# thiery-lab/manifold-mcmc-for-diffusions

Hardware: AMD Instinct MI355X
Metric: constrained-leapfrog steps/sec (all chains), FHN noisy-obs 400 sub-steps (higher is better)
Workload: dtype f64; 1 GPU; FHN noisy-obs, T=100 obs, S=400 steps/obs, R=5 obs/subseq, sigma_y=0.1, 256 chains per GPU (BASELINE.json configs[1]), Newton solver, standard splitting; chains_per_gpu=256, global_chains=256, dim_q=80106, traj_len=16, stepping=chmc_leapfrog_steps per trajectory (batched steps), chain_steps_nominal=152320, parallelism=chains x1 (no data-path collective, 1 gather), ranks_joined=1, collective_world_size=1, collective_route=torch.distributed gather, overlap_halves=-1

## Files before the change

### manifold_mcmc_for_diffusions_amd/csrc/backend_hip.h

```cpp
#pragma once
#include <hip/hip_runtime.h>

static thread_local hipStream_t g_stream = nullptr;
static thread_local hipStream_t g_streams[3] = {nullptr, nullptr, nullptr};
static thread_local int g_device = -1;
static hipError_t g_first_err = hipSuccess;

static inline void note(hipError_t e) {
  if (e != hipSuccess && g_first_err == hipSuccess) g_first_err = e;
}
static int dev_set(int device) {
  hipError_t e = hipSetDevice(device);
  if (e != hipSuccess) {
    g_err = std::string("hipSetDevice: ") + hipGetErrorString(e);
    return -1;
  }
  return 0;
}
static int dev_init(int device) {
  int n = 0;
  hipError_t e = hipGetDeviceCount(&n);
  if (e != hipSuccess || n <= 0) {
    g_err = std::string("no HIP device available (") + hipGetErrorString(e) + ")";
    return -1;
// ... 248 lines not shown
    partial[((size_t)c * gridDim.x + blockIdx.x) * nacc + threadIdx.x] =
        (sm[0][threadIdx.x] + sm[1][threadIdx.x]) + (sm[2][threadIdx.x] + sm[3][threadIdx.x]);
}
static int rowsum_groups(int ncol) { return ((ncol + 1) / 2 + 256 * CHMC_ROWSUM_PAIRS - 1) / (256 * CHMC_ROWSUM_PAIRS); }
template <class F>
static void launch_rowsum(F f, int ncol, int B, int nacc, double* partial, int cls = 0) {
  if (ncol <= 0 || B <= 0) return;
  (void)cls;
  hipLaunchKernelGGL(k_rowsum<F>, dim3((unsigned)rowsum_groups(ncol), (unsigned)B), dim3(256), 0, g_stream, f, ncol, nacc,
                     partial);
  note(hipGetLastError());
}
template <class F>
__global__ void __launch_bounds__(256) k_colmax(F f, int ncol, int rev) {
  const int c = rev ? gridDim.y - 1 - blockIdx.y : blockIdx.y;
  if (!f.active(c)) return;
  const int col = blockIdx.x * 256 + threadIdx.x;
  unsigned long long v = 0ULL;
  if (col < ncol) v = f(c, col);
  unsigned long long* tgt = f.red(c);
  if (!tgt) return;
  for (int off = 32; off > 0; off >>= 1) {
    const unsigned long long o = __shfl_xor(v, off, 64);
    v = o > v ? o : v;
  }
  __shared__ unsigned long long sm[4];
  if ((threadIdx.x & 63) == 0) sm[threadIdx.x >> 6] = v;
  __syncthreads();
  if (threadIdx.x == 0) {
    for (int i = 1; i < 4; ++i) v = sm[i] > v ? sm[i] : v;
    if (v) atomicMax(tgt, v);
  }
}
static thread_local unsigned* g_publish_ticket = nullptr;
template <class F>
static void launch_publish(F f, long n, int* counter, int poll_slot) {
  if (n <= 0) return;
  if (!g_poll_host) {
    note(hipHostMalloc((void**)&g_poll_host, 4 * sizeof(int), hipHostMallocDefault));
    for (int i = 0; i < 4; ++i) note(hipEventCreateWithFlags(&g_poll_ev[i], hipEventDisableTiming));
  }
  if (!g_publish_ticket) {
    note(hipMalloc((void**)&g_publish_ticket, 4 * sizeof(unsigned)));
    note(hipMemset(g_publish_ticket, 0, 4 * sizeof(unsigned)));
  }
  ProfRec r;
  const bool prof = g_prof_on_for(0);
  if (prof) {
    r.a = prof_event(), r.b = prof_event(), r.cls = 0;
    note(hipEventRecord(r.a, g_stream));
  }
  hipLaunchKernelGGL(k_run_publish<F>, dim3((unsigned)((n + 255) / 256)), dim3(256), 0, g_stream, f, (int)n, counter,
                     g_poll_host + poll_slot, g_publish_ticket + poll_slot);
  note(hipGetLastError());
  if (prof) {
    note(hipEventRecord(r.b, g_stream));
    g_prof_pending.push_back(r);
    if (g_prof_pending.size() > 4096) prof_drain();
  }
  note(hipEventRecord(g_poll_ev[poll_slot], g_stream));
}
template <class F>
static void launch_colmax(F f, int ncol, int B, int cls = 0) {
  if (ncol <= 0 || B <= 0) return;
  ProfRec r;
  const bool prof = g_prof_on_for(cls);
  if (prof) {
    r.a = prof_event(), r.b = prof_event(), r.cls = cls;
    note(hipEventRecord(r.a, g_stream));
  }
  hipLaunchKernelGGL(k_colmax<F>, dim3((unsigned)((ncol + 255) / 256), (unsigned)B), dim3(256), 0, g_stream, f, ncol,
                     next_chain_direction());
  note(hipGetLastError());
  if (prof) {
    note(hipEventRecord(r.b, g_stream));
    g_prof_pending.push_back(r);
    if (g_prof_pending.size() > 4096) prof_drain();
  }
}
template <class K, class... Args>
static void launch_wave(K kern, long nwaves, int cls, Args... args) {
  if (nwaves <= 0) return;
  ProfRec r;
  const bool prof = g_prof_on_for(cls);
  if (prof) {
    r.a = prof_event(), r.b = prof_event(), r.cls = cls;
    note(hipEventRecord(r.a, g_stream));
  }
  const int wpb = 1;
  note_forward_launch();
  hipLaunchKernelGGL(kern, dim3((unsigned)((nwaves + wpb - 1) / wpb)), dim3(64 * wpb), 0, g_stream, args...);
  note(hipGetLastError());
  if (prof) {
    note(hipEventRecord(r.b, g_stream));
    g_prof_pending.push_back(r);
    if (g_prof_pending.size() > 4096) prof_drain();
  }
}
template <class K, class... Args>
static void launch_blocks(K kern, long nblocks, int bs, int cls, Args... args) {
  if (nblocks <= 0) return;
  ProfRec r;
  const bool prof = g_prof_on_for(cls);
  if (prof) {
    r.a = prof_event(), r.b = prof_event(), r.cls = cls;
    note(hipEventRecord(r.a, g_stream));
  }
  hipLaunchKernelGGL(kern, dim3((unsigned)nblocks), dim3(bs), 0, g_stream, args...);
  note(hipGetLastError());
  if (prof) {
    note(hipEventRecord(r.b, g_stream));
    g_prof_pending.push_back(r);
// ... 23 lines not shown
```

### manifold_mcmc_for_diffusions_amd/csrc/chmc_api.inc

```
#include <string>
#include <algorithm>
#include <vector>
#include <cstring>
#include <cstdio>
#include <cstdlib>
#include <cmath>
#include <thread>
#include <type_traits>
#include "../../include/chmc.h"
#include "chmc_plan.h"
#include "chmc_layout.h"

using namespace chmc;

static thread_local std::string g_err;
static int fail(const std::string& m) {
  g_err = m;
  return -1;
}
#include CHMC_BACKEND_HEADER

struct chmc_ctx : ChainView {
  std::thread::id owner = std::this_thread::get_id();
  chmc_config cfg;
// ... 372 lines not shown
    launch(KSymBlk<M, RM>{sy, c->sl, c->w, which, 0}, (long)sy.B * sy.K, 9);
    solve_chain<M, RM, 1, 1>(sy, c->sl, c->w, which, 0, psel);
    jt_lambda<M, RM, 1>(c, which, 0, psel);
  });
}

static void iteration_scan(chmc_ctx* c, int newton, int prev, int qsel, int fwd_guess, int use_nw) {
  dispatch(c, [&](auto inst) {
    c->diag[7] += fwd<typename decltype(inst)::M, decltype(inst)::RM>(c, prev ^ 1, qsel, use_nw, newton ? 2 : 0, fwd_guess);
  });
}
static void iteration_scan_pair(chmc_ctx* c, int newton, int prev, int qsel, const Work& w1) {
  dispatch(c, [&](auto inst) {
    c->diag[7] += fwd_pair<typename decltype(inst)::M, decltype(inst)::RM>(c, w1, prev ^ 1, qsel, newton ? 2 : 0);
  });
  c->diag[6]++;
}
static void iteration_after_scan(chmc_ctx* c, int newton, int prev, int qsel) {
  const Sys& sy = c->sy;
  dispatch(c, [&](auto inst) {
    using M = typename decltype(inst)::M;
    constexpr int RM = decltype(inst)::RM;
    bool solved = false;
    if (newton) {
      solved = newton_sweep<M, RM>(c, prev, qsel);
      if (!solved) solve_chain<M, RM, 0, 0>(sy, c->sl, c->w, prev, qsel, 0);
    } else {
      launch(KSymBlk<M, RM>{sy, c->sl, c->w, prev, 1}, (long)sy.B * sy.K, 9);
      solve_chain<M, RM, 1, 0>(sy, c->sl, c->w, prev, qsel, 0);
    }
    jt_lambda<M, RM, 0>(c, prev, qsel, 0, solved);
  });
}

static int retract_waves(const chmc_ctx* c, int newton, const void* views) {
  return chain_kernel_waves(c->plan, part_plan(c).retract_chain && chain_kernel_model(c), c->sy.B, c->num_cus, newton != 0,
                            views != nullptr);
}
static int traj_waves(const chmc_ctx* c, int n_inner, int newton) {
  const bool eligible = part_plan(c).traj_chain && chain_kernel_model(c) && n_inner == 1 && c->mom_tangent && c->halves == 1;
  return chain_kernel_waves(c->plan, eligible, c->sy.B, c->num_cus, newton != 0, false);
}
static int run_projection(chmc_ctx* c, int newton, int prev, int qsel, double ctol, double ptol, double dtol,
                          int max_iters, const ViewSave* views = nullptr, int count_dir = -1) {
  const Sys& sy = c->sy;
  auto iters_dst = [&] { return count_dir < 0 ? nullptr : (count_dir ? c->d_itb : c->d_itf); };
  if (const int waves = retract_waves(c, newton, views)) {
    dispatch(c, [&](auto inst) {
      retract_chain<typename decltype(inst)::M, decltype(inst)::RM>(waves, (long)sy.B, sy, c->sl, c->w, prev, qsel, ctol, ptol,
                                                                     dtol, max_iters, iters_dst());
    });
    c->counters[6]++;
    c->diag[2]++;
    return 0;
  }
  const int nh = views ? 2 : 1;
  auto enter = [&](int h) {
    if (views) set_half(c, *views, h);
  };
  for (int h = 0; h < nh; ++h) {
    enter(h);
    if (sy.B > 0) launch(KNewtonBegin{c->w}, sy.B);
  }
  int fwd_guess = 2;
  const bool carry = c->plan.fwd == FwdPar && sy.K == 1;
  const int max_rounds = carry ? 12 * (max_iters + 1) : max_iters;
// ... 72 lines not shown
  w.Dw = alloc<double>(c, B * KM * RM * RM), w.JuL = alloc<double>(c, B * KM * RM * U), w.zbP = alloc<double>(c, B * KM * RM * Z);
  if (c->plan.pb_allocated) {
    w.muF = alloc<double>(c, B * ivls * X);
    w.ivl = alloc<double>(c, B * ivls * (2 * X * X + X * Z));
  }
  w.err = alloc<double>(c, B), w.ndq = alloc<unsigned long long>(c, B);
  w.iters = alloc<int>(c, B), w.nw = alloc<int>(c, B), w.nstat = alloc<int>(c, B), w.ok = alloc<int>(c, B), w.status = alloc<int>(c, B);
  w.n_active = alloc<int>(c, 4);
  c->d_itf_next = alloc<int>(c, B);
  c->have_pair = true;
}

static int run_projection_pair(chmc_ctx* c, int newton, double ctol, double ptol, double dtol, int max_iters) {
  const Sys& sy = c->sy;
  const int prev = 1, qsel = 1;
  const Work wk[2] = {c->w, c->pw};
  int* const iters_dst[2] = {c->d_itb, c->d_itf_next};
  const int dir[2] = {1, 0};
  auto enter = [&](int p) { c->w = wk[p]; };
  bool done[2], predict[2], stopped[2] = {false, false};
  int rounds_done[2] = {0, 0};
  for (int p = 0; p < 2; ++p) {
    enter(p);
    launch(KNewtonBegin{c->w}, sy.B);
    done[p] = sy.B <= 0;
    predict[p] = c->proj_stable[dir[p]] >= 3 && c->proj_rounds[dir[p]] >= 2;
  }
  for (int it = 0; it < max_iters && !(done[0] && done[1]); ++it) {
    for (int p = 0; p < 2; ++p)
      if (!done[p] && predict[p] && it >= c->proj_rounds[dir[p]] && poll_end(2 * p + ((it - 1) & 1)) == 0)
        done[p] = stopped[p] = true;
    if (done[0] && done[1]) break;
    c->round = it;
    if (!done[0] && !done[1]) {
      enter(0);
      iteration_scan_pair(c, newton, prev, qsel, wk[1]);
    } else {
      enter(done[0] ? 1 : 0);
      iteration_scan(c, newton, prev, qsel, it == 0 ? 2 : 1, 1);
    }
    for (int p = 0; p < 2; ++p) {
      if (done[p]) continue;
      enter(p);
      iteration_after_scan(c, newton, prev, qsel);
      const KCheck chk{c->w, ctol, ptol, dtol, max_iters, sy.B, iters_dst[p], it & 3};
      if (it >= 1) launch_publish(chk, sy.B, c->w.n_active + (it & 3), 2 * p + (it & 1));
      else launch(chk, sy.B);
      c->counters[6]++, c->diag[8]++;
    }
    if (it == 0) continue;
    for (int p = 0; p < 2; ++p) {
      if (done[p]) continue;
      if (it >= 2 && poll_end(2 * p + ((it - 1) & 1)) == 0) {
        done[p] = true;
        c->counters[6]--;
        continue;
      }
      rounds_done[p] = it + 1;
      if (it + 1 >= max_iters) poll_end(2 * p + (it & 1));
    }
  }
  for (int p = 0; p < 2; ++p) {
    int& expect = c->proj_rounds[dir[p]];
    int& stable = c->proj_stable[dir[p]];
    if (stopped[p] && rounds_done[p] < expect) rounds_done[p] = expect;
    stable = rounds_done[p] == expect ? stable + 1 : 0;
    expect = rounds_done[p];
    enter(p);
    if (sy.B > 0) launch(KNewtonEnd{c->w, iters_dst[p]}, sy.B);
  }
  enter(0);
  c->round = 0;
  return 0;
}

static int check_ctx(const chmc_ctx* c, const char* fn) {
  if (!c) return fail(std::string(fn) + ": null context");
// ... 1312 lines not shown
```

### manifold_mcmc_for_diffusions_amd/csrc/chmc_core.h

```cpp
#pragma once
#include <math.h>
#include <stdint.h>
#include "chmc_model.h"

#define CHMC_FI __attribute__((always_inline))
#if defined(__HIPCC__)
#define CHMC_UNROLL _Pragma("unroll")
#define CHMC_UNROLL4 _Pragma("unroll 4")
#else
#define CHMC_UNROLL
#define CHMC_UNROLL4
#endif

namespace chmc {

#ifndef CHMC_FWD_DEPTH
#define CHMC_FWD_DEPTH 4
#endif
#define CHMC_Q_PAD 256
#define CHMC_TPAD 16

struct BlockDesc {
  int obs0, nobs, first, last;
  int row0, nrows, ny;
// ... 1616 lines not shown
        const double* lam = w.lampad + ((size_t)c * sy.Kmax + b) * RM;
        const double* lam2 = w.lampad2 + ((size_t)c * sy.Kmax + b) * RM;
        const double* Jv = pick(sl.Jv, s) + (size_t)c * RM * sy.NV + col;
        const int nr = sy.blk[b].nrows;
        for (int i = 0; i < RM; ++i)
          if (i < nr) {
            const double jv = Jv[(size_t)i * sy.NV];
            d += jv * lam[i];
            if (TGT == 3) d2 += jv * lam2[i];
          }
      } else {
        const int t = e - sy.V0;
        col = sy.NV + t;
        const int b = sy.obs2blk[t];
        const int j = t - sy.blk[b].obs0;
        if (j < sy.blk[b].ny) {
          const double sg = sigma_at(sy, pick(sl.q, s) + (size_t)c * sy.Q);
          d = sg * w.lampad[((size_t)c * sy.Kmax + b) * RM + j];
          if (TGT == 3) d2 = sg * w.lampad2[((size_t)c * sy.Kmax + b) * RM + j];
        }
      }
      if (TGT == 0) r = absbits(d);
      const double gn = tgt[col] - d;
      tgt[col] = gn;
      if (TGT == 3) {
        const double pn = tgt2[col] - d2;
        tgt2[col] = pn;
        if (flow_rev) rev_flow1(c, s, off + col, pn, gn);
      }
    }
    return r;
  }
};

template <class M>
struct KInitInterp {
  Sys sy;
  double* q;
  const double* u;
  const double* v0;
  const double* xobs;
  CHMC_HD void operator()(int tid) const {
    constexpr int X = M::X, V = M::V;
    static_assert(X == V, "the interpolation solve needs a square noise matrix");
    const int TS = sy.T * sy.S;
    const int c = tid / TS, s = tid - c * TS;
    const int t = s / sy.S, i = s - t * sy.S;
    double* qc = q + (size_t)c * sy.Q;
    const double* uc = u + (size_t)c * sy.U;
    ChainConsts<M> cc;
    cc.init(uc, sy.dl);
    double xa[X], xs[X], dlt[X], f0[X], zero[V], A[X * X], Bm[X * V], rhs[X];
    if (t == 0) {
      M::gx0(cc.z, v0 + (size_t)c * sy.V0, xa);
    } else {
      for (int a = 0; a < X; ++a) xa[a] = xobs[((size_t)c * sy.T + t - 1) * X + a];
    }
    for (int a = 0; a < X; ++a) {
      dlt[a] = (xobs[((size_t)c * sy.T + t) * X + a] - xa[a]) / sy.S;
      xs[a] = xa[a] + i * dlt[a];
    }
    for (int a = 0; a < V; ++a) zero[a] = 0.0;
    M::step(cc.k, xs, zero, f0);
    M::jac_ab(cc.k, xs, zero, A, Bm);
    for (int a = 0; a < X; ++a) rhs[a] = dlt[a] - (f0[a] - xs[a]);
    int piv[X];
// ... 1076 lines not shown
```

### manifold_mcmc_for_diffusions_amd/csrc/chmc_passes.inc

```

static_assert(SirModel::ID == CHMC_MODEL_SIR && SirVsModel::ID == CHMC_MODEL_SIR && FhnModel::ID == CHMC_MODEL_FHN &&
                  FhnVsModel::ID == CHMC_MODEL_FHN && FhnNbModel::ID == CHMC_MODEL_FHN_NOTEBOOK,
              "chain_kernel_model and kChainKernels gate the per-chain kernels on the same models");
static bool chain_kernel_model(const chmc_ctx* c) { return c->model == CHMC_MODEL_SIR; }
template <class M, int RM>
constexpr bool kChainKernels = RM == 16 && M::ID == CHMC_MODEL_SIR;

template <int RM, int TGT>
static void update(const Sys& sy, const Slots& sl, const Work& w, int which, int qsel, int psel) {
  if (sy.Q % 2 == 0 && sy.NV % 2 == 0 && sy.U % 2 == 0 && sy.V0 % 2 == 0 && sy.V % 2 == 0 && sy.NCOL % 2 == 0)
    launch_colmax(KUpdate<RM, TGT, 2>{sy, sl, w, which, qsel, psel}, sy.NCOL / 2, sy.B, 4);
  else
    launch_colmax(KUpdate<RM, TGT, 1>{sy, sl, w, which, qsel, psel}, sy.NCOL, sy.B, 4);
}
template <class M, int RM, int TGT>
static void jt_lambda(chmc_ctx* c, int which, int qsel, int psel, bool have_mu_f = false, int flow_rev = 0,
                      double* fwd_qb = nullptr, double fwd_hfrac = 0.0) {
  const Sys& sy = c->sy;
  if (c->plan.rows != RowsCompact) return update<RM, TGT>(sy, c->sl, c->w, which, qsel, psel);
  if (!have_mu_f) launch(KMuF<RM, M::X, TGT>{sy, c->sl, c->w, which}, (long)sy.B * sy.K * sy.NOBS * M::X, 5);
  launch_colmax(KUpdatePB<RM, M::X, M::V, TGT>{sy, c->sl, c->w, which, qsel, psel, flow_rev, fwd_qb, fwd_hfrac},
                sy.T * sy.S + sy.V0 + (sy.noisy ? sy.T : 0), sy.B, 4);
}

// ... 156 lines not shown
        launch_blocks(k_newton_ivl<M>, nbk * sy.NOBS, 64, 1, sy, c->sl, c->w, prev, qsel);
        launch_blocks(k_newton_comb<M, RM>, nbk, 64, 1, sy, c->sl, c->w, prev, qsel);
        break;
      case Newton16LdsrowsGramMfma:
        launch_blocks(k_rev_wave_ldsrows<M, RM, 1>, nbk, 64, 1, sy, c->sl, c->w, prev, qsel);
        launch_blocks(k_gram_rows_mfma<RM>, nbk, 64, 1, sy, c->sl, c->w, prev, 1, qsel), c->diag[0]++;
        break;
      default:
        launch_blocks(k_rev_wave_ldsrows<M, RM, 1>, nbk, 64, 1, sy, c->sl, c->w, prev, qsel);
        launch_wave(k_gram_rows<RM, 4>, nbk * (RM / 4), 1, sy, c->sl, c->w, prev, 1, qsel), c->diag[1]++;
    }
    if (!solved) launch_blocks(k_newton_factor_wave<M, RM>, (nbk + 3) / 4, 64, 9, sy, c->sl, c->w, prev, qsel);
  } else {
    switch (sweep) {
      case NewtonIvlFsm:
      case NewtonIvlComb:
        launch_blocks(k_newton_ivl<M>, nbk * sy.NOBS, 64, 1, sy, c->sl, c->w, prev, qsel);
        launch_blocks(k_newton_comb<M, RM>, nbk, 64, 1, sy, c->sl, c->w, prev, qsel);
        break;
      case NewtonRevStoreGramMfma:
        launch_wave(k_rev_wave<M, RM, 1, false>, nbk, 1, sy, c->sl, c->w, prev, qsel);
        launch_blocks(k_gram_rows_mfma<RM>, nbk, 64, 1, sy, c->sl, c->w, prev, 1, qsel), c->diag[0]++;
        break;
      default:
        launch_wave(k_rev_wave<M, RM, 1>, nbk, 1, sy, c->sl, c->w, prev, qsel);
    }
    if (solved)
      launch_blocks(k_newton_fsm_wave<M, RM>, (long)sy.B, 64, 5, sy, c->sl, c->w, prev, qsel), c->diag[4]++;
    else
      launch(KNewtonFactor<M, RM>{sy, c->sl, c->w, prev}, nbk, 9), c->diag[5]++;
  }
  return solved;
}

template <class M, int RM>
static void jw(chmc_ctx* c, int which, int vsel, bool compact) {
  const Sys& sy = c->sy;
  if (compact)
    launch_wave(k_jw_pb<RM, M::X, M::V>, (long)sy.B * sy.K, 6, sy, c->sl, c->w, which, vsel);
  else
    launch_wave(k_jw_wave<RM>, (long)sy.B * sy.K, 6, sy, c->sl, c->w, which, vsel);
}
static void project_pair(chmc_ctx* c, int which, bool fix_in_jw, bool flow_rev, double* fwd_qb, double fwd_hfrac) {
  const Sys& sy = c->sy;
  dispatch(c, [&](auto inst) {
    using M = typename decltype(inst)::M;
    constexpr int RM = decltype(inst)::RM;
    switch (part_plan(c).jp) {
      case JpPbWg:
        if constexpr (RM > 8)
          launch_blocks(k_jw_pb_wg<RM, M::X, M::V, CHMC_RETRACT_WAVES>, (long)sy.B, 64 * CHMC_RETRACT_WAVES, 6, sy, c->sl, c->w,
                        which);
        break;
      case JpPb:
        if constexpr (RM <= 8 && M::V == 2) {
          if (fix_in_jw) {
            launch_wave(k_jw_pb<RM, M::X, M::V, true, true>, (long)sy.B * sy.K, 6, sy, c->sl, c->w, which, 256);
            break;
          }
        }
        launch_wave(k_jw_pb<RM, M::X, M::V, true>, (long)sy.B * sy.K, 6, sy, c->sl, c->w, which, 256);
        break;
      case JpWave:
        launch_wave(k_jw_wave<RM, true>, (long)sy.B * sy.K, 6, sy, c->sl, c->w, which, 256);
        break;
    }
// ... 61 lines not shown

template <class M, int RM, int SYM, int TGT>
static void solve_chain(const Sys& sy, const Slots& sl, const Work& w, int which, int qsel, int psel) {
  launch(KSolveChain<M, RM, SYM, TGT>{sy, sl, w, which, qsel, psel}, sy.B, 5);
}
template <class M, int RM>
static int fwd(chmc_ctx* c, int which, int qsel, int use_nw, int store, int) {
  if (store) return 0;
  launch(KFwd<M, RM>{c->sy, c->sl, c->w, which, qsel, use_nw, store}, (long)c->sy.B * c->sy.K, 7);
  return 1;
}
template <class M, int RM>
static int fwd_pair(chmc_ctx* c, const Work& w1, int which, int qsel, int store) {
  const Sys& sy = c->sy;
  if (store) return 0;
  launch(KFwd<M, RM>{sy, c->sl, c->w, which, qsel, 1, store}, (long)sy.B * sy.K, 7);
  launch(KFwd<M, RM>{sy, c->sl, w1, which, qsel, 1, store}, (long)sy.B * sy.K, 7);
  return 2;
}
template <class M, int RM>
static void state_sweep(chmc_ctx* c, int which) {
  launch(KStateBlk<M, RM>{c->sy, c->sl, c->w, which}, (long)c->sy.B * c->sy.K, 2);
}
template <class M, int RM>
static void gld_sweeps(chmc_ctx* c, int which) {
  launch(KGldBlk<M, RM>{c->sy, c->sl, c->w, which}, (long)c->sy.B * c->sy.K, 3);
}
template <class M, int RM>
static bool newton_sweep(chmc_ctx* c, int prev, int qsel) {
  launch(KNewtonBlk<M, RM>{c->sy, c->sl, c->w, prev, qsel}, (long)c->sy.B * c->sy.K, 1);
  return false;
}
template <class M, int RM>
static void jw(chmc_ctx* c, int which, int vsel, bool) {
  launch(KJw<RM>{c->sy, c->sl, c->w, which, vsel}, (long)c->sy.B * c->sy.K * RM, 6);
}
static void project_momentum(chmc_ctx* c, int which, int vsel, int psel);
static void project_pair(chmc_ctx* c, int which, bool, bool, double*, double) {
  project_momentum(c, which, 0, 0);
  project_momentum(c, which, 4, 3);
}
template <class M>
static void gd_grad(chmc_ctx* c, long tasks, const double* q, const double* cres, double reg_coeff, double* g, double* part) {
  launch(KGdGrad<M>{c->sy, q, c->w.trajw, cres, reg_coeff, g, part}, tasks);
}
template <class M>
static void xobs_par(chmc_ctx*) { no_wave_kernels("the partition switch's time-parallel pass"); }
template <class M, int RM>
static void nld_sweeps(chmc_ctx*, const Sys&, int, int, double*) { no_wave_kernels("the comparator target"); }
template <class M, int RM, class... Args>
static void retract_chain(int, long, Args...) { no_wave_kernels("the per-chain retraction"); }
template <class M, int RM, class... Args>
static void traj_chain(int, long, Args...) { no_wave_kernels("the per-chain trajectory"); }
#endif
```

### manifold_mcmc_for_diffusions_amd/csrc/chmc_plan.h

```cpp
#pragma once
#include <climits>
#include <cstdlib>

#ifndef CHMC_RETRACT_WAVES
#define CHMC_RETRACT_WAVES 8
#endif
#ifndef CHMC_CHAIN_SCAN_WAVES
#define CHMC_CHAIN_SCAN_WAVES 4
#endif
static_assert(CHMC_CHAIN_SCAN_WAVES == 1 || CHMC_CHAIN_SCAN_WAVES == 2 || CHMC_CHAIN_SCAN_WAVES == 4,
              "k_fwd_par is launched with 1, 2 or 4 wavefronts per workgroup (fwd_par in chmc_passes.inc)");
#ifndef CHMC_CHAIN_WG4_MAX_PER_CU
#define CHMC_CHAIN_WG4_MAX_PER_CU 4
#endif

namespace chmc {

constexpr int kSwitchUnset = INT_MIN;
struct Switches {
  bool compact_rows = true, gram_mfma = false;
  int par_scan = kSwitchUnset, par_waves = kSwitchUnset, row_split = 0, halves = 1;
  bool no_fwd_scan = false, step_fusions = true;
  int retract_kernel = kSwitchUnset, pair_retract = kSwitchUnset;
};
inline Switches read_switches() {
  auto env = [](const char* name, int unset) {
    const char* e = getenv(name);
    return e ? atoi(e) : unset;
  };
  static const bool compact_rows = env("CHMC_COMPACT_ROWS", 1) != 0, gram_mfma = env("CHMC_GRAM_MFMA", 0) != 0;
  Switches s;
  s.compact_rows = compact_rows, s.gram_mfma = gram_mfma;
  s.par_scan = env("CHMC_PAR_SCAN", kSwitchUnset), s.par_waves = env("CHMC_PAR_WAVES", kSwitchUnset);
  s.row_split = env("CHMC_ROW_SPLIT", 0), s.halves = env("CHMC_HALVES", 1);
  s.no_fwd_scan = getenv("CHMC_NO_FWD_SCAN") != nullptr, s.step_fusions = env("CHMC_STEP_FUSIONS", 1) != 0;
  s.retract_kernel = env("CHMC_RETRACT_KERNEL", kSwitchUnset);
  s.pair_retract = env("CHMC_PAIR_RETRACT", kSwitchUnset);
  return s;
}

struct PlanInput {
  int rmt;
  int num_partition;
  int K[2];
  int longest;
  int chain_steps;
  bool s_tiles8;
  int V;
  bool even_dims;
  bool gaussian;
  bool wave_kernels;
  Switches sw;
  Switches call;
};

enum RowFamily { RowsCompact, RowsStored, RowsStoredMfma };
enum FwdScan { FwdPar , FwdWave , FwdFunctor  };
enum StateSweep {
  StateLean,
  StateIvlComb,
  StateIvlCombWg,
  StateLdsrowsGram,
  StateLdsrowsGramMfma,
  StateRevWave,
  StateRevStoreGramMfma
};
enum NewtonSweep {
  NewtonIvlFsm,
  NewtonIvlComb,
  NewtonRevWave,
// ... 5 lines not shown
  Newton16LdsrowsGramMfma
};
enum GldSweep {
  GldQxLean,
  GldIvl,
  GldCompactFwdStored,
  GldStored
};
enum JpPass { JpPb , JpPbWg , JpWave  };

struct PartitionPlan {
  StateSweep state;
  NewtonSweep newton;
  GldSweep gld;
  JpPass jp;
  bool rebuild_rows;
  bool retract_chain;
  bool traj_chain;
};
struct KernelPlan {
  RowFamily rows;
  bool pb_allocated;
  bool par_scan;
  FwdScan fwd;
  FwdScan fwd_cold;
  int fwd_waves;
  FwdScan nld;
  int nld_waves;
  bool mom_fix_in_jp;
  bool rev_flow_in_update;
  int retract_kernel;
  bool pair_retractions;
  int pair_retract;
  PartitionPlan part[2];
};

inline int par_waves_for(int env, long longest) {
  if (env == 1 || env == 2 || env == 4) return env;
  return longest >= 4096 ? 4 : longest >= 2048 ? 2 : 1;
}
inline bool few_long_blocks(int nblocks_per_chain, long longest) { return nblocks_per_chain <= 4 && longest >= 1024; }

inline KernelPlan make_plan(const PlanInput& in) {
  const Switches& sw = in.sw;
  KernelPlan pl{};
  const bool rows16 = in.rmt > 8;
  const int kmax = in.K[0] > in.K[in.num_partition - 1] ? in.K[0] : in.K[in.num_partition - 1];
  const bool chain16_layout = kmax == 1 && rows16;

  const bool compact = in.wave_kernels && sw.compact_rows && !sw.gram_mfma;
  pl.rows = compact ? RowsCompact : sw.gram_mfma ? RowsStoredMfma : RowsStored;
  pl.pb_allocated = compact || (in.wave_kernels && sw.compact_rows && rows16);

  pl.par_scan = sw.par_scan != kSwitchUnset ? sw.par_scan != 0
                                            : few_long_blocks(kmax, in.longest) || (chain16_layout && sw.compact_rows && !sw.gram_mfma);
  pl.fwd_waves = chain16_layout && sw.par_waves == kSwitchUnset ? CHMC_CHAIN_SCAN_WAVES : par_waves_for(sw.par_waves, in.longest);
  pl.fwd_cold = in.wave_kernels && in.s_tiles8 && !in.call.no_fwd_scan ? FwdWave : FwdFunctor;
  pl.fwd = in.wave_kernels && pl.par_scan ? FwdPar : pl.fwd_cold;
  const bool nld_par = in.call.par_scan != kSwitchUnset ? in.call.par_scan != 0 : few_long_blocks(1, in.chain_steps);
  pl.nld = nld_par ? FwdPar : in.s_tiles8 ? FwdWave : FwdFunctor;
  pl.nld_waves = par_waves_for(in.call.par_waves, in.chain_steps);

  const bool step_fusions = pl.pb_allocated && in.call.step_fusions && !rows16;
  pl.mom_fix_in_jp = step_fusions && in.V == 2 && in.even_dims;
  pl.rev_flow_in_update = step_fusions && !in.gaussian;
  pl.retract_kernel = in.call.retract_kernel;
  pl.pair_retract = in.call.pair_retract;
  pl.pair_retractions = in.call.pair_retract != 0 && sw.halves != 2 && pl.fwd != FwdPar &&
                        (!in.wave_kernels || pl.fwd_cold == FwdWave || in.call.pair_retract == 1);

  for (int p = 0; p < in.num_partition; ++p) {
    PartitionPlan& pp = pl.part[p];
    const int K = in.K[p];
    const bool split = sw.row_split == 1 ? false : (sw.row_split == 2 || sw.row_split == 4) ? true : K <= 4;
    const bool ivl16 = rows16 && compact && split;
    const bool chain16 = chain16_layout && ivl16;
    if (rows16) {
      pp.state = chain16 ? StateIvlCombWg : ivl16 ? StateIvlComb : sw.gram_mfma ? StateLdsrowsGramMfma : StateLdsrowsGram;
      pp.newton = chain16 ? Newton16IvlCombWg
                  : compact ? (K == 1 ? Newton16IvlCombFactor : Newton16IvlComb)
                  : sw.gram_mfma ? Newton16LdsrowsGramMfma : Newton16LdsrowsGram;
      pp.gld = ivl16 ? GldIvl : compact ? GldCompactFwdStored : GldStored;
    } else {
      pp.state = compact ? StateLean : sw.gram_mfma ? StateRevStoreGramMfma : StateRevWave;
      pp.newton = compact ? (K <= 64 ? NewtonIvlFsm : NewtonIvlComb) : sw.gram_mfma ? NewtonRevStoreGramMfma : NewtonRevWave;
      pp.gld = compact ? GldQxLean : GldStored;
    }
    pp.jp = chain16 ? JpPbWg : compact ? JpPb : JpWave;
    pp.rebuild_rows = compact && (!rows16 || ivl16);
    pp.retract_chain = compact && rows16 && K == 1;
    pp.traj_chain = pp.retract_chain && ivl16;
    if (pp.retract_chain) pl.pair_retractions = false;
  }
  return pl;
}

inline int chain_kernel_waves(const KernelPlan& pl, bool eligible, int B, int num_cus, bool newton, bool half_batches) {
  if (!eligible || !newton || half_batches) return 0;
  const int want = pl.retract_kernel != kSwitchUnset ? pl.retract_kernel
                   : B <= num_cus ? 1 : B <= CHMC_CHAIN_WG4_MAX_PER_CU * num_cus ? 2 : 0;
  return want == 1 ? CHMC_RETRACT_WAVES : want == 2 ? 4 : 0;
}

inline bool pair_this_call(const KernelPlan& pl, bool wave_kernels, int B, int K, int num_cus) {
  if (!pl.pair_retractions) return false;
  if (pl.pair_retract == 1 || !wave_kernels) return true;
  return 2 * (((long)B * K + 63) / 64) <= num_cus;
}

}
```

### manifold_mcmc_for_diffusions_amd/csrc/chmc_wave.h

```cpp
#pragma once
#include <type_traits>
#include "chmc_core.h"

namespace chmc {

#ifdef CHMC_PLAIN_STREAM
__device__ inline double ld_stream(const double* p) { return *p; }
#else
__device__ inline double ld_stream(const double* p) { return __builtin_nontemporal_load(p); }
#endif

__device__ __forceinline__ void st_async(double* p, double v) {
  asm volatile("global_store_dwordx2 %0, %1, off\n\ts_nop 1" : : "v"(p), "v"(v) : "memory");
}
__device__ __forceinline__ void st_async2(double* p, double v0, double v1) {
  typedef double d2v __attribute__((ext_vector_type(2)));
  const d2v v = {v0, v1};
  asm volatile("global_store_dwordx4 %0, %1, off\n\ts_nop 1" : : "v"(p), "v"(v) : "memory");
}

__device__ inline double bcast0(double x) {
  union { double d; int i[2]; } u;
  u.d = x;
  u.i[0] = __builtin_amdgcn_readfirstlane(u.i[0]);
// ... 1157 lines not shown
  }
  double* out = w.ivl + (cb * sy.NOBS + m) * CHMC_IVL_N(X, Z);
#pragma unroll
  for (int i = 0; i < X * X; ++i) {
    double v = Sacc[i];
#pragma unroll
    for (int o = 32; o > 0; o >>= 1) v += __shfl_xor(v, o, 64);
    if (lane == 0) out[i] = v;
  }
#pragma unroll
  for (int i = 0; i < X * Z; ++i) {
    double v = Wacc[i];
#pragma unroll
    for (int o = 32; o > 0; o >>= 1) v += __shfl_xor(v, o, 64);
    if (lane == 0) out[X * X + i] = v;
  }
  if (lane == 0) {
#pragma unroll
    for (int i = 0; i < X * X; ++i) out[X * X + X * Z + i] = Pf[i];
  }
}
template <class M, bool STATE = false>
__global__ void __launch_bounds__(64, CHMC_IVL_WAVES) k_newton_ivl(Sys sy, Slots sl, Work w, int which, int qsel) {
  const int wid = blockIdx.x;
  if (wid >= sy.B * sy.K * sy.NOBS) return;
  const int m = wid % sy.NOBS;
  const int cbi = sy.order[wid / sy.NOBS];
  const int c = cbi / sy.K, b = cbi - c * sy.K;
  if (STATE ? !w.ok[c] : !newton_select(w, c, which, qsel)) return;
  const BlockDesc bd = sy.blk[b];
  if (m >= bd.nobs) return;
  newton_ivl_body<M, STATE>(sy, sl, w, which, qsel, c, b, m, bd);
}

template <class M, int RM, bool STATE, bool FACTOR>
__device__ __forceinline__ void newton_comb_body(const Sys& sy, const Slots& sl, const Work& w, int which, int qsel, int c, int b,
                                                 const BlockDesc& bd) {
  constexpr int X = M::X, Z = M::Z, U = M::U, V0 = M::V0;
  constexpr int NI = CHMC_IVL_N(X, Z);
  static_assert(!(STATE && FACTOR), "the factor step belongs to a Newton iteration");
  __shared__ double LamF[RM * X], LamN[RM * X], Dl[RM * RM], zl[RM * Z], Ys[RM * X], Iv[NI], JuS[FACTOR ? RM * M::U : 1];
  const int lane = threadIdx.x & 63;
  const int sl_ = sl.cur[c] ^ which;
  const size_t cb = (size_t)c * sy.Kmax + b;
  const int S = sy.S, NV = sy.NV;
  const double* q = (STATE ? pick(sl.q, sl_) : (qsel ? w.qb : pick(sl.q, sl_ ^ 1))) + (size_t)c * sy.Q;
  const double* traj = (STATE ? pick(sl.traj, sl_) : w.trajw) + (size_t)c * sy.TRJ + (size_t)(bd.step0 + CHMC_TPAD * b) * X;
  double* Jr = pick(sl.Jv, sl_) + (size_t)c * RM * NV;
  double* LFr = pick(sl.LF, sl_) + cb * sy.NOBS * RM * X;
  auto lds_sync = [&]() {
    __builtin_amdgcn_fence(__ATOMIC_ACQ_REL, "workgroup");
    __builtin_amdgcn_wave_barrier();
  };
  for (int e = lane; e < RM * X; e += 64) LamF[e] = 0.0;
  for (int e = lane; e < RM * RM; e += 64) Dl[e] = 0.0;
  for (int e = lane; e < RM * Z; e += 64) zl[e] = 0.0;
  lds_sync();
  for (int m = bd.nobs - 1; m >= 0; --m) {
    if (m < bd.ny) {
      double g[X], gl = 0.0;
      M::obs_grad(traj + (size_t)(m + 1) * S * X, g);
#pragma unroll
      for (int a = 0; a < X; ++a) gl = lane == a ? g[a] : gl;
      if (lane < X) LamF[m * X + lane] = gl;
    }
    if (m == bd.nobs - 1 && !bd.last) {
// ... 82 lines not shown
  for (int e = lane; e < RM * U; e += 64) {
    const int i = e / U, d = e - i * U;
    double tt = 0.0;
    if (d < Z) {
      for (int mz = 0; mz < Z; ++mz) {
        double gs = 0.0;
#pragma unroll
        for (int ee = 0; ee < Z * Z; ++ee) gs = ee == mz * Z + d ? G[ee] : gs;
        tt += zl[i * Z + mz] * gs;
      }
    } else {
      tt = i < bd.ny ? sigma_at(sy, q) * q[sy.U + sy.NV + bd.obs0 + i] : 0.0;
    }
    if constexpr (FACTOR) JuS[e] = tt;
    else (STATE ? pick(sl.JuP, sl_) : w.JuL)[cb * RM * U + e] = tt;
  }
  if constexpr (STATE) {
    for (int e = lane; e < RM * Z; e += 64) w.zbP[cb * RM * Z + e] = zl[e];
  }
  if constexpr (FACTOR) {
    lds_sync();
    newton_factor16<M, RM, true>(sy, sl, w, which, qsel, c, b, lane < 16, Dl, JuS);
  }
}
template <class M, int RM, bool STATE = false, bool FACTOR = false>
__global__ void __launch_bounds__(64) k_newton_comb(Sys sy, Slots sl, Work w, int which, int qsel) {
  const int wid = blockIdx.x;
  if (wid >= sy.B * sy.K) return;
  const int cbi = sy.order[wid];
  const int c = cbi / sy.K, b = cbi - c * sy.K;
  if (STATE ? !w.ok[c] : !newton_select(w, c, which, qsel)) return;
  const BlockDesc bd = sy.blk[b];
  newton_comb_body<M, RM, STATE, FACTOR>(sy, sl, w, which, qsel, c, b, bd);
}

template <class M, int RM, int MODE>
__global__ void __launch_bounds__(64) k_rev_wave_ldsrows(Sys sy, Slots sl, Work w, int which, int qsel) {
  constexpr int X = M::X, V = M::V, Z = M::Z, U = M::U, V0 = M::V0;
  __shared__ double LamS[RM * X];
  __shared__ double zaccS[RM * Z * 64];
  const int lane = threadIdx.x & 63;
  const int wid = blockIdx.x;
  if (wid >= sy.B * sy.K) return;
  const int cbi = sy.order[wid];
  const int c = cbi / sy.K, b = cbi - c * sy.K;
  if (MODE == 1 ? !newton_select(w, c, which, qsel) : !w.ok[c]) return;
  const BlockDesc bd = sy.blk[b];
  const int sl_ = sl.cur[c] ^ which;
  const size_t cb = (size_t)c * sy.Kmax + b;
  const int S = sy.S, NV = sy.NV;
  const double* q = (MODE == 1 ? (qsel ? w.qb : pick(sl.q, sl_ ^ 1)) : pick(sl.q, sl_)) + (size_t)c * sy.Q;
  const double* traj = (MODE == 1 ? w.trajw : pick(sl.traj, sl_)) + (size_t)c * sy.TRJ + (size_t)(bd.step0 + CHMC_TPAD * b) * X;
  double* Jo = (MODE == 1 ? w.JvW : pick(sl.Jv, sl_)) + (size_t)c * RM * NV;
  ChainConsts<M> cc;
  cc.init(q, sy.dl);
  const double* vbase = q + sy.U + sy.V0 + (size_t)bd.step0 * V;
  const size_t colb = (size_t)sy.V0 + (size_t)bd.step0 * V;
  auto lds_sync = [&]() {
    __builtin_amdgcn_fence(__ATOMIC_ACQ_REL, "workgroup");
    __builtin_amdgcn_wave_barrier();
  };
  for (int i = lane; i < RM * X; i += 64) LamS[i] = 0.0;
  for (int i = 0; i < RM * Z; ++i) zaccS[i * 64 + lane] = 0.0;
  lds_sync();
  double* PBo = nullptr;
  double* LFo = nullptr;
// ... 2640 lines not shown
#pragma unroll
    for (int k = 0; k < RM; ++k)
      if (k > i) t -= L[k * RM + i] * x[k];
    x[i] = t / L[i * RM + i];
  }
  if (!act) return;
#pragma unroll
  for (int i = 0; i < RM; ++i) {
    double t = 0.0;
#pragma unroll
    for (int a = 0; a < U; ++a) t += Ws[g][i * U + a] * e[a];
    const double v = (i >= nrows || r >= nrows) ? 0.0 : x[i] - t;
    w.gMb[cb * RM * RM + i * RM + r] = v;
  }
  double Gz[Z * Z];
  M::gz_jac(pick(sl.q, s) + (size_t)c * sy.Q, Gz);
#pragma unroll
  for (int d = 0; d < U; ++d) w.gWu[(cb * RM + r) * U + d] = wu[d];
#pragma unroll
  for (int mz = 0; mz < Z; ++mz) {
    double t = 0.0;
#pragma unroll
    for (int d = 0; d < Z; ++d) t += Gz[mz * Z + d] * wu[d];
    w.gzd[(cb * RM + r) * Z + mz] = t;
  }
}
template <class M, int RM>
__global__ void __launch_bounds__(64) k_gld_prep_wave(Sys sy, Slots sl, Work w, int which) {
  gld_prep_body<M, RM>(sy, sl, w, which, blockIdx.x * 4, 4);
}


template <class M, int RM>
__global__ void __launch_bounds__(64) k_newton_fsm_wave(Sys sy, Slots sl, Work w, int prev, int qsel) {
  constexpr int U = M::U, X = M::X;
  static_assert(RM <= 8, "one block per lane: the RM x RM matrix lives in registers");
  const int lane = threadIdx.x & 63;
  const int c = blockIdx.x;
  if (c >= sy.B) return;
  if (!newton_select(w, c, prev, qsel)) return;
  const int sp = sl.cur[c] ^ prev;
  const bool has = lane < sy.K;
  const size_t cb = (size_t)c * sy.Kmax + (has ? lane : 0);
  double D[RM * RM], JuL[RM * U], cp[RM];
  unsigned long long eb = 0ULL;
#pragma unroll
  for (int i = 0; i < RM * RM; ++i) D[i] = has ? w.Dw[cb * RM * RM + i] : ((i / RM == i % RM) ? 1.0 : 0.0);
#pragma unroll
  for (int i = 0; i < RM * U; ++i) JuL[i] = has ? w.JuL[cb * RM * U + i] : 0.0;
#pragma unroll
  for (int i = 0; i < RM; ++i) {
    cp[i] = has ? w.cpad[cb * RM + i] : 0.0;
    const unsigned long long vb = absbits(cp[i]);
    eb = vb > eb ? vb : eb;
  }
  {
    int piv[RM];
    lu_factor<RM>(D, piv);
    lu_solve<RM, 1>(D, piv, cp);
    lu_solve<RM, U>(D, piv, JuL);
  }
  const double* jur = pick(sl.JuP, sp) + cb * RM * U;
  double ju[RM * U];
#pragma unroll
  for (int i = 0; i < RM * U; ++i) ju[i] = has ? jur[i] : 0.0;
  double sacc[U], Cm[U * U];
#pragma unroll
  for (int a = 0; a < U; ++a) {
    double t2 = 0.0;
#pragma unroll
    for (int i = 0; i < RM; ++i) t2 += ju[i * U + a] * cp[i];
    sacc[a] = has ? t2 : 0.0;
#pragma unroll
// ... 65 lines not shown
    const BlockDesc bd = sy.blk[lane];
    const double* lfb = pick(sl.LF, sp) + cb * sy.NOBS * RM * X;
    double* mo = w.muF + cb * sy.NOBS * X;
    for (int m0 = 0; m0 < sy.NOBS; m0 += 4) {
      double t4[4][X], lf[4][RM * X];
#pragma unroll
      for (int k = 0; k < 4; ++k) {
        const bool in = m0 + k < sy.NOBS;
#pragma unroll
        for (int e = 0; e < RM * X; ++e) lf[k][e] = in ? lfb[(m0 + k) * RM * X + e] : 0.0;
      }
#pragma unroll
      for (int k = 0; k < 4; ++k) {
        const int m = m0 + k;
#pragma unroll
        for (int a = 0; a < X; ++a) {
          double t = 0.0;
          if (m < bd.nobs) {
#pragma unroll
            for (int i = 0; i < RM; ++i)
              if (i < bd.nrows) t += lam[i] * lf[k][i * X + a];
          }
          t4[k][a] = t;
        }
      }
#pragma unroll
      for (int k = 0; k < 4; ++k)
        if (m0 + k < sy.NOBS) {
#pragma unroll
          for (int a = 0; a < X; ++a) mo[(m0 + k) * X + a] = t4[k][a];
        }
    }
  }
}

template <class M, int RM, bool FUSE = false>
__global__ void __launch_bounds__(64) k_newton_factor_wave(Sys sy, Slots sl, Work w, int prev, int qsel) {
  const int lane = threadIdx.x & 63;
  const int tid = blockIdx.x * 4 + (lane >> 4);
  const bool live = tid < sy.B * sy.K;
  const int tc = live ? tid : 0;
  const int c = tc / sy.K, b = tc - c * sy.K;
  const bool act = newton_select(w, c, prev, qsel) && live;
  const size_t cb = (size_t)c * sy.Kmax + b;
  newton_factor16<M, RM, FUSE>(sy, sl, w, prev, qsel, c, b, act, w.Dw + cb * RM * RM, w.JuL + cb * RM * M::U);
}

typedef double d2_t __attribute__((ext_vector_type(2)));
template <int OFF>
__device__ __forceinline__ void vm_load16(d2_t& dst, const void* p) {
  asm volatile("global_load_dwordx4 %0, %1, off offset:%2" : "=v"(dst) : "v"(p), "n"(OFF) : "memory");
}
template <int I, int N, int OFF0>
struct TileLoad {
  static __device__ __forceinline__ void run(d2_t* r, const void* p) {
    vm_load16<OFF0 + 16 * I>(r[I], p);
    TileLoad<I + 1, N, OFF0>::run(r, p);
  }
};
template <int N, int OFF0>
struct TileLoad<N, N, OFF0> {
  static __device__ __forceinline__ void run(d2_t*, const void*) {}
};
template <int NOUT>
__device__ __forceinline__ void vm_wait(d2_t (&r)[8]) {
  asm volatile("s_waitcnt vmcnt(%8)"
// ... 810 lines not shown
```

Before: 55450 steps/s.

## Merge forward and backward Newton passes into paired kernel launches

When both projection directions are still iterating under the Newton solver, the interval, combine, FSM and Jt-lambda update passes for the two work sets now run as single paired launches. Previously each direction ran its own sequence. The aim is to halve kernel launch count and per-launch overhead and to fill the GPU better with two problems per grid. The merge is controlled by a plan switch (on by default, gated on pair retractions, wave kernels, compact rows and the IvlFsm Newton mode). It adds duplicated kernel code, and the paired update reads the PB data once for both directions.

```diff
diff --git a/manifold_mcmc_for_diffusions_amd/csrc/backend_hip.h b/manifold_mcmc_for_diffusions_amd/csrc/backend_hip.h
--- a/manifold_mcmc_for_diffusions_amd/csrc/backend_hip.h
+++ b/manifold_mcmc_for_diffusions_amd/csrc/backend_hip.h
@@ -304,6 +304,33 @@
     if (v) atomicMax(tgt, v);
   }
 }
+template <class F>
+__global__ void __launch_bounds__(256) k_colmax_pair(F f, int ncol, int rev) {
+  const int c = rev ? gridDim.y - 1 - blockIdx.y : blockIdx.y;
+  const int act = f.active(c);
+  if (!act) return;
+  const int col = blockIdx.x * 256 + threadIdx.x;
+  unsigned long long v[2] = {0ULL, 0ULL};
+  if (col < ncol) f(c, col, act, v);
+  __shared__ unsigned long long sm[2][4];
+#pragma unroll
+  for (int p = 0; p < 2; ++p) {
+    for (int off = 32; off > 0; off >>= 1) {
+      const unsigned long long o = __shfl_xor(v[p], off, 64);
+      v[p] = o > v[p] ? o : v[p];
+    }
+    if ((threadIdx.x & 63) == 0) sm[p][threadIdx.x >> 6] = v[p];
+  }
+  __syncthreads();
+  if (threadIdx.x == 0) {
+#pragma unroll
+    for (int p = 0; p < 2; ++p) {
+      unsigned long long m = v[p];
+      for (int i = 1; i < 4; ++i) m = sm[p][i] > m ? sm[p][i] : m;
+      if (((act >> p) & 1) && m) atomicMax(f.red(c, p), m);
+    }
+  }
+}
 static thread_local unsigned* g_publish_ticket = nullptr;
 template <class F>
 static void launch_publish(F f, long n, int* counter, int poll_slot) {
@@ -350,6 +377,24 @@
     if (g_prof_pending.size() > 4096) prof_drain();
   }
 }
+template <class F>
+static void launch_colmax_pair(F f, int ncol, int B, int cls = 0) {
+  if (ncol <= 0 || B <= 0) return;
+  ProfRec r;
+  const bool prof = g_prof_on_for(cls);
+  if (prof) {
+    r.a = prof_event(), r.b = prof_event(), r.cls = cls;
+    note(hipEventRecord(r.a, g_stream));
+  }
+  hipLaunchKernelGGL(k_colmax_pair<F>, dim3((unsigned)((ncol + 255) / 256), (unsigned)B), dim3(256), 0, g_stream, f, ncol,
+                     next_chain_direction());
+  note(hipGetLastError());
+  if (prof) {
+    note(hipEventRecord(r.b, g_stream));
+    g_prof_pending.push_back(r);
+    if (g_prof_pending.size() > 4096) prof_drain();
+  }
+}
 template <class K, class... Args>
 static void launch_wave(K kern, long nwaves, int cls, Args... args) {
   if (nwaves <= 0) return;
diff --git a/manifold_mcmc_for_diffusions_amd/csrc/chmc_api.inc b/manifold_mcmc_for_diffusions_amd/csrc/chmc_api.inc
--- a/manifold_mcmc_for_diffusions_amd/csrc/chmc_api.inc
+++ b/manifold_mcmc_for_diffusions_amd/csrc/chmc_api.inc
@@ -428,6 +428,15 @@
     jt_lambda<M, RM, 0>(c, prev, qsel, 0, solved);
   });
 }
+static void iteration_after_scan_pair(chmc_ctx* c, int prev, int qsel, const Work& w1) {
+  dispatch(c, [&](auto inst) {
+    using M = typename decltype(inst)::M;
+    constexpr int RM = decltype(inst)::RM;
+    newton_sweep_pair<M, RM>(c, w1, prev, qsel);
+    jt_lambda_pair<M, RM>(c, w1, prev, qsel);
+  });
+  c->diag[9]++;
+}
 
 static int retract_waves(const chmc_ctx* c, int newton, const void* views) {
   return chain_kernel_waves(c->plan, part_plan(c).retract_chain && chain_kernel_model(c), c->sy.B, c->num_cus, newton != 0,
@@ -566,9 +575,12 @@
         done[p] = stopped[p] = true;
     if (done[0] && done[1]) break;
     c->round = it;
-    if (!done[0] && !done[1]) {
+    const bool both = !done[0] && !done[1];
+    const bool merged = both && newton && c->plan.pair_passes;
+    if (both) {
       enter(0);
       iteration_scan_pair(c, newton, prev, qsel, wk[1]);
+      if (merged) iteration_after_scan_pair(c, prev, qsel, wk[1]);
     } else {
       enter(done[0] ? 1 : 0);
       iteration_scan(c, newton, prev, qsel, it == 0 ? 2 : 1, 1);
@@ -576,7 +588,7 @@
     for (int p = 0; p < 2; ++p) {
       if (done[p]) continue;
       enter(p);
-      iteration_after_scan(c, newton, prev, qsel);
+      if (!merged) iteration_after_scan(c, newton, prev, qsel);
       const KCheck chk{c->w, ctol, ptol, dtol, max_iters, sy.B, iters_dst[p], it & 3};
       if (it >= 1) launch_publish(chk, sy.B, c->w.n_active + (it & 3), 2 * p + (it & 1));
       else launch(chk, sy.B);
diff --git a/manifold_mcmc_for_diffusions_amd/csrc/chmc_core.h b/manifold_mcmc_for_diffusions_amd/csrc/chmc_core.h
--- a/manifold_mcmc_for_diffusions_amd/csrc/chmc_core.h
+++ b/manifold_mcmc_for_diffusions_amd/csrc/chmc_core.h
@@ -1672,6 +1672,117 @@
     return r;
   }
 };
+template <int RM, int X, int V>
+struct KUpdatePBPair {
+  Sys sy;
+  Slots sl;
+  Work w, w1;
+  int which, qsel;
+  CHMC_HD int active(int c) const {
+    int p_ = 0, q_ = 0;
+    return (newton_select(w, c, p_, q_) ? 1 : 0) | (newton_select(w1, c, p_, q_) ? 2 : 0);
+  }
+  CHMC_HD unsigned long long* red(int c, int p) const { return p ? &w1.ndq[c] : &w.ndq[c]; }
+  CHMC_FI CHMC_HD void operator()(int c, int idx, int act, unsigned long long (&r)[2]) const {
+    const int s = sl.cur[c] ^ which;
+    const size_t off = (size_t)c * sy.Q + sy.U;
+    double* tgt[2] = {(qsel ? w.qb : pick(sl.q, s ^ 1)) + off, (qsel ? w1.qb : pick(sl.q, s ^ 1)) + off};
+    const bool on[2] = {(act & 1) != 0, (act & 2) != 0};
+    const int TS = sy.T * sy.S;
+    r[0] = r[1] = 0ULL;
+    if (idx < TS) {
+      const int st0 = idx;
+      const int g = st0 / sy.S;
+      const int b = sy.obs2blk[g];
+      const int m = g - sy.blk[b].obs0;
+      const size_t mo = (((size_t)c * sy.Kmax + b) * sy.NOBS + m) * X;
+      const double* pb = pick(sl.PB, s) + ((size_t)c * TS + st0) * (X * V);
+      const size_t to = sy.V0 + (size_t)st0 * V;
+      const bool wide = V == 2 && !((sy.Q | sy.U | sy.V0) & 1);
+      double old[2][V], pbv[X * V], mu[2][X];
+      CHMC_UNROLL
+      for (int p = 0; p < 2; ++p) {
+        if (!on[p]) continue;
+        if (wide) {
+          const double2_ o = *reinterpret_cast<const double2_*>(tgt[p] + to);
+          old[p][0] = o.x, old[p][V - 1] = o.y;
+        } else {
+          CHMC_UNROLL
+          for (int k = 0; k < V; ++k) old[p][k] = tgt[p][to + k];
+        }
+      }
+      if ((X * V) % 2 == 0) {
+        CHMC_UNROLL
+        for (int k = 0; k < X * V; k += 2) {
+          const double2_ v = ld2_stream(pb + k);
+          pbv[k] = v.x, pbv[k + 1 < X * V ? k + 1 : k] = v.y;
+        }
+      } else {
+        CHMC_UNROLL
+        for (int k = 0; k < X * V; ++k) pbv[k] = pb[k];
+      }
+      CHMC_UNROLL
+      for (int a = 0; a < X; ++a) {
+        if (on[0]) mu[0][a] = w.muF[mo + a];
+        if (on[1]) mu[1][a] = w1.muF[mo + a];
+      }
+      CHMC_UNROLL
+      for (int p = 0; p < 2; ++p) {
+        if (!on[p]) continue;
+        CHMC_UNROLL
+        for (int k = 0; k < V; ++k) {
+          double tt = 0.0;
+          CHMC_UNROLL
+          for (int a = 0; a < X; ++a) tt += mu[p][a] * pbv[a * V + k];
+          const unsigned long long vb = absbits(tt);
+          r[p] = vb > r[p] ? vb : r[p];
+          old[p][k] -= tt;
+        }
+        if (wide) {
+          double2_ o;
+          o.x = old[p][0], o.y = old[p][V - 1];
+          *reinterpret_cast<double2_*>(tgt[p] + to) = o;
+        } else {
+          CHMC_UNROLL
+          for (int k = 0; k < V; ++k) tgt[p][to + k] = old[p][k];
+        }
+      }
+    } else {
+      const int e = idx - TS;
+      CHMC_UNROLL
+      for (int p = 0; p < 2; ++p) {
+        if (!on[p]) continue;
+        const double* lampad = p ? w1.lampad : w.lampad;
+        double d = 0.0;
+        int col;
+        if (e < sy.V0) {
+          col = e;
+          const int b = sy.obs2blk[0];
+          const double* lam = lampad + ((size_t)c * sy.Kmax + b) * RM;
+          const double* Jv = pick(sl.Jv, s) + (size_t)c * RM * sy.NV + col;
+          const int nr = sy.blk[b].nrows;
+          for (int i = 0; i < RM; ++i)
+            if (i < nr) {
+              const double jv = Jv[(size_t)i * sy.NV];
+              d += jv * lam[i];
+            }
+        } else {
+          const int t = e - sy.V0;
+          col = sy.NV + t;
+          const int b = sy.obs2blk[t];
+          const int j = t - sy.blk[b].obs0;
+          if (j < sy.blk[b].ny) {
+            const double sg = sigma_at(sy, pick(sl.q, s) + (size_t)c * sy.Q);
+            d = sg * lampad[((size_t)c * sy.Kmax + b) * RM + j];
+          }
+        }
+        r[p] = absbits(d);
+        const double gn = tgt[p][col] - d;
+        tgt[p][col] = gn;
+      }
+    }
+  }
+};
 
 template <class M>
 struct KInitInterp {
diff --git a/manifold_mcmc_for_diffusions_amd/csrc/chmc_passes.inc b/manifold_mcmc_for_diffusions_amd/csrc/chmc_passes.inc
--- a/manifold_mcmc_for_diffusions_amd/csrc/chmc_passes.inc
+++ b/manifold_mcmc_for_diffusions_amd/csrc/chmc_passes.inc
@@ -212,6 +212,23 @@
   }
   return solved;
 }
+template <class M, int RM>
+static void newton_sweep_pair(chmc_ctx* c, const Work& w1, int prev, int qsel) {
+  const Sys& sy = c->sy;
+  const long nbk = (long)sy.B * sy.K;
+  if constexpr (RM <= 8) {
+    launch_blocks(k_newton_ivl_pair<M>, nbk * sy.NOBS, 128, 1, sy, c->sl, c->w, prev, qsel, w1);
+    launch_blocks(k_newton_comb_pair<M, RM>, 2 * nbk, 64, 1, sy, c->sl, c->w, prev, qsel, w1);
+    launch_blocks(k_newton_fsm_wave_pair<M, RM>, 2 * (long)sy.B, 64, 5, sy, c->sl, c->w, prev, qsel, w1), c->diag[4]++;
+  }
+}
+template <class M, int RM>
+static void jt_lambda_pair(chmc_ctx* c, const Work& w1, int prev, int qsel) {
+  const Sys& sy = c->sy;
+  if constexpr (RM <= 8)
+    launch_colmax_pair(KUpdatePBPair<RM, M::X, M::V>{sy, c->sl, c->w, w1, prev, qsel}, sy.T * sy.S + sy.V0 + (sy.noisy ? sy.T : 0),
+                       sy.B, 4);
+}
 
 template <class M, int RM>
 static void jw(chmc_ctx* c, int which, int vsel, bool compact) {
@@ -339,6 +356,23 @@
   return false;
 }
 template <class M, int RM>
+static void newton_sweep_pair(chmc_ctx* c, const Work& w1, int prev, int qsel) {
+  const Work w0 = c->w;
+  for (int p = 0; p < 2; ++p) {
+    c->w = p ? w1 : w0;
+    if (!newton_sweep<M, RM>(c, prev, qsel)) solve_chain<M, RM, 0, 0>(c->sy, c->sl, c->w, prev, qsel, 0);
+  }
+  c->w = w0;
+}
+template <class M, int RM>
+static void jt_lambda_pair(chmc_ctx* c, const Work& w1, int prev, int qsel) {
+  const Work w0 = c->w;
+  jt_lambda<M, RM, 0>(c, prev, qsel, 0);
+  c->w = w1;
+  jt_lambda<M, RM, 0>(c, prev, qsel, 0);
+  c->w = w0;
+}
+template <class M, int RM>
 static void jw(chmc_ctx* c, int which, int vsel, bool) {
   launch(KJw<RM>{c->sy, c->sl, c->w, which, vsel}, (long)c->sy.B * c->sy.K * RM, 6);
 }
diff --git a/manifold_mcmc_for_diffusions_amd/csrc/chmc_plan.h b/manifold_mcmc_for_diffusions_amd/csrc/chmc_plan.h
--- a/manifold_mcmc_for_diffusions_amd/csrc/chmc_plan.h
+++ b/manifold_mcmc_for_diffusions_amd/csrc/chmc_plan.h
@@ -22,6 +22,7 @@
   int par_scan = kSwitchUnset, par_waves = kSwitchUnset, row_split = 0, halves = 1;
   bool no_fwd_scan = false, step_fusions = true;
   int retract_kernel = kSwitchUnset, pair_retract = kSwitchUnset;
+  bool pair_passes = true;
 };
 inline Switches read_switches() {
   auto env = [](const char* name, int unset) {
@@ -36,6 +37,7 @@
   s.no_fwd_scan = getenv("CHMC_NO_FWD_SCAN") != nullptr, s.step_fusions = env("CHMC_STEP_FUSIONS", 1) != 0;
   s.retract_kernel = env("CHMC_RETRACT_KERNEL", kSwitchUnset);
   s.pair_retract = env("CHMC_PAIR_RETRACT", kSwitchUnset);
+  s.pair_passes = env("CHMC_PAIR_PASSES", 1) != 0;
   return s;
 }
 
@@ -107,6 +109,7 @@
   int retract_kernel;
   bool pair_retractions;
   int pair_retract;
+  bool pair_passes;
   PartitionPlan part[2];
 };
 
@@ -167,6 +170,8 @@
     pp.traj_chain = pp.retract_chain && ivl16;
     if (pp.retract_chain) pl.pair_retractions = false;
   }
+  pl.pair_passes = pl.pair_retractions && in.call.pair_passes && in.wave_kernels && pl.rows == RowsCompact && in.rmt <= 8;
+  for (int p = 0; p < in.num_partition; ++p) pl.pair_passes = pl.pair_passes && pl.part[p].newton == NewtonIvlFsm;
   return pl;
 }
 
diff --git a/manifold_mcmc_for_diffusions_amd/csrc/chmc_wave.h b/manifold_mcmc_for_diffusions_amd/csrc/chmc_wave.h
--- a/manifold_mcmc_for_diffusions_amd/csrc/chmc_wave.h
+++ b/manifold_mcmc_for_diffusions_amd/csrc/chmc_wave.h
@@ -1213,6 +1213,20 @@
   if (m >= bd.nobs) return;
   newton_ivl_body<M, STATE>(sy, sl, w, which, qsel, c, b, m, bd);
 }
+template <class M>
+__global__ void __launch_bounds__(128, CHMC_IVL_WAVES) k_newton_ivl_pair(Sys sy, Slots sl, Work w0, int which, int qsel, Work w1) {
+  const int wid = blockIdx.x;
+  if (wid >= sy.B * sy.K * sy.NOBS) return;
+  const bool second = __builtin_amdgcn_readfirstlane(threadIdx.x >> 6) != 0;
+  const Work w = second ? w1 : w0;
+  const int m = wid % sy.NOBS;
+  const int cbi = sy.order[wid / sy.NOBS];
+  const int c = cbi / sy.K, b = cbi - c * sy.K;
+  if (!newton_select(w, c, which, qsel)) return;
+  const BlockDesc bd = sy.blk[b];
+  if (m >= bd.nobs) return;
+  newton_ivl_body<M, false>(sy, sl, w, which, qsel, c, b, m, bd);
+}
 
 template <class M, int RM, bool STATE, bool FACTOR>
 __device__ __forceinline__ void newton_comb_body(const Sys& sy, const Slots& sl, const Work& w, int which, int qsel, int c, int b,
@@ -1361,6 +1375,19 @@
   if (STATE ? !w.ok[c] : !newton_select(w, c, which, qsel)) return;
   const BlockDesc bd = sy.blk[b];
   newton_comb_body<M, RM, STATE, FACTOR>(sy, sl, w, which, qsel, c, b, bd);
+}
+template <class M, int RM>
+__global__ void __launch_bounds__(64) k_newton_comb_pair(Sys sy, Slots sl, Work w0, int which, int qsel, Work w1) {
+  const int n = sy.B * sy.K;
+  const bool second = (int)blockIdx.x >= n;
+  const int wid = second ? (int)blockIdx.x - n : (int)blockIdx.x;
+  if (wid >= n) return;
+  const Work w = second ? w1 : w0;
+  const int cbi = sy.order[wid];
+  const int c = cbi / sy.K, b = cbi - c * sy.K;
+  if (!newton_select(w, c, which, qsel)) return;
+  const BlockDesc bd = sy.blk[b];
+  newton_comb_body<M, RM, false, false>(sy, sl, w, which, qsel, c, b, bd);
 }
 
 template <class M, int RM, int MODE>
@@ -4067,13 +4094,10 @@
 
 
 template <class M, int RM>
-__global__ void __launch_bounds__(64) k_newton_fsm_wave(Sys sy, Slots sl, Work w, int prev, int qsel) {
+__device__ __forceinline__ void newton_fsm_body(const Sys& sy, const Slots& sl, const Work& w, int prev, int qsel, int c) {
   constexpr int U = M::U, X = M::X;
   static_assert(RM <= 8, "one block per lane: the RM x RM matrix lives in registers");
   const int lane = threadIdx.x & 63;
-  const int c = blockIdx.x;
-  if (c >= sy.B) return;
-  if (!newton_select(w, c, prev, qsel)) return;
   const int sp = sl.cur[c] ^ prev;
   const bool has = lane < sy.K;
   const size_t cb = (size_t)c * sy.Kmax + (has ? lane : 0);
@@ -4205,6 +4229,22 @@
         }
     }
   }
+}
+template <class M, int RM>
+__global__ void __launch_bounds__(64) k_newton_fsm_wave(Sys sy, Slots sl, Work w, int prev, int qsel) {
+  const int c = blockIdx.x;
+  if (c >= sy.B) return;
+  if (!newton_select(w, c, prev, qsel)) return;
+  newton_fsm_body<M, RM>(sy, sl, w, prev, qsel, c);
+}
+template <class M, int RM>
+__global__ void __launch_bounds__(64) k_newton_fsm_wave_pair(Sys sy, Slots sl, Work w0, int prev, int qsel, Work w1) {
+  const bool second = (int)blockIdx.x >= sy.B;
+  const int c = second ? (int)blockIdx.x - sy.B : (int)blockIdx.x;
+  if (c >= sy.B) return;
+  const Work w = second ? w1 : w0;
+  if (!newton_select(w, c, prev, qsel)) return;
+  newton_fsm_body<M, RM>(sy, sl, w, prev, qsel, c);
 }
 
 template <class M, int RM, bool FUSE = false>
```

After: 60230 steps/s, median of 6. 1.09x the previous value.
